# wearepal/qBOLD-VI

Measured on AMD Instinct MI355X. Metric: voxel-ELBO evals/sec, higher is better.
Workload: dtype f32; 1 GPU; 1048576 synthetic voxels/GPU x 11 tau, S=32 likelihood draws, K=70 KL draws, encoder U=60, L=2 (optimal.yaml), fused qbold_vi_fwd, tissue integral: table; encoder arithmetic: operands split in two f16 halves, three MFMA passes (hi.hi, hi.lo, lo.hi), f32 accumulate: float32-grade (~22 significant bits), |x| < 65504; sampling, forward model and ELBO sums: f32; global_voxels=1048576, parallelism=voxel-shard x1, collective=none

## Files before the change

### qbold_vi_amd/csrc/elbo_core.h

```cpp
#pragma once
#ifndef QB_PRIO_LIK
#define QB_PRIO_LIK 1
#endif
#ifndef QB_LIK_BARRIER
#define QB_LIK_BARRIER 2
#endif
#ifndef QB_GT_DEPTH
#define QB_GT_DEPTH 8
#endif
#ifndef QB_GT_DEPTH_LONG
#define QB_GT_DEPTH_LONG 2
#endif
#ifndef QB_X_DEPTH
#define QB_X_DEPTH 2
#endif
#ifndef QB_PRIO_KL
#define QB_PRIO_KL 2
#endif
#ifndef QB_PRIO_AFTER
#define QB_PRIO_AFTER 0
#endif

#include "qbold_dev.h"

// ... 76 lines not shown
    k.mask = mask;
}

template <int T, int SE, bool LITERAL>
__device__ __forceinline__ float sample_nll(const FwdLds* L, const QbDev& c, const VoxelLik<T>& k,
                                            float oef, float dbv) {
    const FwdVox fv = fwd_vox(c, oef, dbv);
    float s[T];
    if (SE >= 0) {
        constexpr int kSE = SE >= 0 ? SE : 0;
        float tis[T];
#pragma unroll
        for (int t = T - 1; t >= 0; --t) {
            const int m = (t < kSE && 2 * kSE - t < T) ? 2 * kSE - t : 0;
            const bool mirrored = t < kSE && 2 * kSE - t < T && c.full_model && c.taus[m] == -c.taus[t];
            if (mirrored) tis[t] = tis[m];
            else tis[t] = fwd_tissue<LITERAL>(L, c, fv, t);
            s[t] = fwd_mix(c, fv, tis[t], t);
        }
    } else {
#pragma unroll
        for (int t = 0; t < T; ++t) s[t] = fwd_signal<LITERAL>(L, c, fv, t);
    }
    const float inv_np = 1.0f / se_norm<T, SE>(c, s);
    float acc = 0.0f;
#pragma unroll
    for (int t = 0; t < T; ++t) {
        float yp = s[t] * inv_np;
        if (c.predict_log) yp = k.mask > 0.0f ? __logf(yp) : 0.0f;
        float r = (k.yt[t] - yp) * k.inv_s[t];
        if (c.use_student_t)
            acc += 0.5f * (c.st_df + 1.0f) * log1pf(r * r / c.st_df) - c.st_const;
        else
            acc = fmaf(0.5f * r, r, acc);
    }
    return acc + k.log_s_sum;
}

template <class LDS>
struct IsGtLds { static constexpr bool value = false; };
template <int T, int SE>
struct IsGtLds<GtLds<T, SE>> { static constexpr bool value = true; };

template <bool HELD>
struct GtStage {
    float4 kk;
    float bb;
};
template <>
struct GtStage<true> {
    float4 kk;
};

template <int T, int SE, class U = NoDrawRegs>
__device__ __forceinline__ float sample_sq_fast(const GtLds<T, SE>* L, const QbDev& c, const VoxelLik<T>& k,
                                                float sa, float sb, const U& u = U()) {
    static_assert(SE >= 0 && gtab_segs(T) > 0, "built for compile-time spin-echo protocols");
    static_assert(!U::kOn || !gtab_paired(T, SE), "held draw operands: built for the unpaired table");
    constexpr int NSEG = gtab_segs(T);
    FwdFast fv;
    float bb_se;
    if constexpr (U::kOn) {
        fv = fwd_fast_sig(u, sa, sb);
        bb_se = u.bb[SE];
    } else {
        fv = fwd_fast_sig(c, sa, sb);
        bb_se = L->blood_B[SE];
    }
    float acc = 0.0f;
    const float s_se = fmaf(fv.tissue_w, 1.0f, fv.blood_w * exp2f_(fv.ng * bb_se));
    const float inv_np = rcpf_(s_se + 1e-3f);
    const float lt = log2f_(fv.tissue_w * inv_np), lb = log2f_(fv.blood_w * inv_np);
    static_assert(QB_GT_OEF_MIN == QB_MIN_OEF && QB_GT_OEF_RANGE == QB_OEF_RANGE, "the table spans forward_transform's range");
    const float cg = fminf(sa * (float)NSEG, (float)NSEG - 0.0009765625f);
    const float f = __builtin_amdgcn_fractf(cg);
    const float4* row = L->gtab + (int)cg;
    {
        const float r = fmaf(-(s_se * inv_np), k.inv_s[SE], k.yt[SE]);
        acc = fmaf(r, r, acc);
    }
    constexpr int NA = T - 1 - SE, NB = (2 * SE - (T - 1)) > 0 ? 2 * SE - (T - 1) : 0, NE = NA + NB;
    auto score = [&](int t, float yh) {
        const float r = fmaf(-yh, k.inv_s[t], k.yt[t]);
        acc = fmaf(r, r, acc);
    };
    if constexpr (gtab_paired(T, SE)) {
        typedef float f32x2 __attribute__((ext_vector_type(2)));
        static_assert(NB == 0 && NA % 2 == 0, "paired table: every evaluated tau above the spin echo, in pairs");
        struct Stage {
            float4 A, B;
            f32x2 bb;
        };
        auto issue = [&](int p) -> Stage {
            Stage st;
            st.A = row[(2 * p) * NSEG];
            st.B = row[(2 * p + 1) * NSEG];
            st.bb = f32x2{L->blood_B[SE + 1 + 2 * p], L->blood_B[SE + 2 + 2 * p]};
            return st;
        };
        const f32x2 ff{f, f}, nd2{fv.nd, fv.nd}, ng2{fv.ng, fv.ng}, lt2{lt, lt}, lb2{lb, lb};
        auto finish = [&](int p, const Stage& st) {
            const f32x2 c0{st.A.x, st.A.y}, c1{st.A.z, st.A.w}, c2{st.B.x, st.B.y}, c3{st.B.z, st.B.w};
            const f32x2 F = __builtin_elementwise_fma(__builtin_elementwise_fma(__builtin_elementwise_fma(c3, ff, c2), ff, c1), ff, c0);
            const f32x2 e1 = __builtin_elementwise_fma(nd2, F, lt2), e2 = __builtin_elementwise_fma(ng2, st.bb, lb2);
            score(SE + 1 + 2 * p, exp2f_(e1.x) + exp2f_(e2.x));
            score(SE + 2 + 2 * p, exp2f_(e1.y) + exp2f_(e2.y));
        };
        constexpr int NP = NA / 2;
        constexpr int D = (QB_GT_DEPTH + 1) / 2 < NP ? (QB_GT_DEPTH + 1) / 2 : NP;
        Stage ring[D + 1];
#pragma unroll
        for (int e = 0; e < D; ++e) ring[e] = issue(e);
#pragma unroll
        for (int e = 0; e < NP; ++e) {
            if (e + D < NP) ring[(e + D) % (D + 1)] = issue(e + D);
            __builtin_amdgcn_sched_barrier(0);
            finish(e, ring[e % (D + 1)]);
            __builtin_amdgcn_sched_barrier(0);
        }
        return acc;
    } else {
        using Stage = GtStage<U::kOn>;
        auto issue = [&](int t) -> Stage {
            const int j = t > SE ? t - SE : SE - t;
            Stage st;
            st.kk = row[(j - 1) * NSEG];
            if constexpr (!U::kOn) st.bb = L->blood_B[t];
            return st;
        };
// ... 116 lines not shown
    bool whitened;
    if constexpr (LPV == 1) whitened = zk == nullptr && row_all(reach < QB_LOGIT_CLIP);
    else whitened = zk == nullptr && __all(reach < QB_LOGIT_CLIP);
    if (whitened) {
        const float dmu_o = q.mu_o - prior.mu_o, dmu_d = q.mu_d - prior.mu_d;
        const float d0 = dmu_o * prior.i_so, m00 = q.e_so * prior.i_so;
        const float d1 = fmaf(dmu_d, prior.i_sd, dmu_o * prior.i_bl);
        const float m10 = fmaf(q.c, prior.i_sd, q.e_so * prior.i_bl), m11 = q.e_sd * prior.i_sd;
        float s0 = 0.0f, s1 = 0.0f, s00 = 0.0f, s11 = 0.0f, s01 = 0.0f;
        for (int g = part; 4 * g < K; g += QB_LANES_PER_VOXEL) {
            float z[8];
            const int cnt = K - 4 * g < 4 ? K - 4 * g : 4;
            n_kl += cnt;
            normals8_unscaled(seed, vox, (uint32_t)g, STREAM_KL, cnt, z);
#pragma unroll
            for (int d = 0; d < 4; ++d) {
                s0 += z[2 * d];
                s1 += z[2 * d + 1];
                s00 = fmaf(z[2 * d], z[2 * d], s00);
                s11 = fmaf(z[2 * d + 1], z[2 * d + 1], s11);
                s01 = fmaf(z[2 * d], z[2 * d + 1], s01);
            }
        }
        s0 *= QB_BM_K;
        s1 *= QB_BM_K;
        s00 *= QB_BM_K * QB_BM_K;
        s11 *= QB_BM_K * QB_BM_K;
        s01 *= QB_BM_K * QB_BM_K;
        const float nk = (float)n_kl;
        const float quad = fmaf(fmaf(m00, m00, m10 * m10) - 1.0f, s00, fmaf(fmaf(m11, m11, -1.0f), s11, 2.0f * m10 * m11 * s01));
        const float lin = 2.0f * fmaf(fmaf(d0, m00, d1 * m10), s0, d1 * m11 * s1);
        return fmaf(nk, fmaf(d0, d0, d1 * d1), lin + quad);
    }
    for (int g = part; 4 * g < K; g += QB_LANES_PER_VOXEL) {
        const int cnt = K - 4 * g < 4 ? K - 4 * g : 4;
        n_kl += cnt;
        DrawQuad dq;
        if (!zk) dq.load(seed, vox, (uint32_t)g, STREAM_KL);
#pragma unroll 1
        for (int d = 0; d < cnt; ++d) {
            float z0, z1;
            if (zk) {
                z0 = zk[2 * (4 * g + d)];
                z1 = zk[2 * (4 * g + d) + 1];
            } else {
                dq.next(z0, z1);
            }
            kl_sum += kl_swr_diff(q, prior, z0, z1);
        }
    }
    return kl_sum;
}

template <int T, int SE, bool FAST, bool LITERAL, bool MIR, class LDS, class U = NoDrawRegs>
__device__ __forceinline__ float lik_draws(const LDS* L, const QbDev& c, const VoxelLik<T>& lik, const LogitMvn& q,
                                           int S, const float* __restrict__ zs, uint64_t seed, uint64_t vox, int part,
                                           int& n_lik, const U& u = U()) {
    static_assert(!U::kOn || (FAST && IsGtLds<LDS>::value), "held draw operands: the per-tau-table fast path");
    float nll_sum = 0.0f;
    const int calls = S > 4 * part ? (S - 4 * part + 15) / 16 : 0;
    const int last = calls > 0 ? S - 4 * (part + 4 * (calls - 1)) : 0;
    n_lik = calls > 0 ? 4 * (calls - 1) + (last < 4 ? last : 4) : 0;
    DrawQuad dq;
    uint32_t g = (uint32_t)part;
#pragma unroll 1
    for (int i = 0; i < n_lik; ++i) {
        float z0, z1;
        if (zs) {
            const int draw = 4 * (part + 4 * (i >> 2)) + (i & 3);
            z0 = zs[2 * draw];
            z1 = zs[2 * draw + 1];
        } else {
            if ((i & 3) == 0) {
                dq.load(seed, vox, g, STREAM_LIK);
                g += QB_LANES_PER_VOXEL;
            }
            dq.next(z0, z1);
        }
        float a, b, oef = 0.0f, dbv = 0.0f;
        reparam_logits(q, z0, z1, a, b);
        if constexpr (!(FAST && IsGtLds<LDS>::value)) forward_transform(a, b, oef, dbv);
        if constexpr (U::kOn) {
            nll_sum += sample_sq_fast<T, SE>(L, c, lik, sigmoidf_(a), sigmoidf_(b), u);
        } else if constexpr (FAST && IsGtLds<LDS>::value) {
            static_assert(!IsGtLds<LDS>::value || MIR, "the per-tau table scores merged mirror pairs");
            nll_sum += sample_sq_fast<T, SE>(L, c, lik, sigmoidf_(a), sigmoidf_(b));
        } else if constexpr (FAST) {
            nll_sum += sample_sq_fast<T, SE, MIR>(L, c, lik, oef, dbv);
        } else {
            nll_sum += sample_nll<T, SE, LITERAL>(L, c, lik, oef, dbv);
        }
    }
    return nll_sum;
}

__device__ __forceinline__ void share_sum(int p, float v, float& first, float& pair) {
    pair = (p & 1) ? pair + v : v;
    first = p == 1 ? pair : first;
}

template <int T, int SE, bool FAST, bool LITERAL, bool MIR = false, int LPV = QB_LANES_PER_VOXEL, bool DREGS = false,
          class LDS>
__device__ __forceinline__ void voxel_mc_sums(const LDS* L, const QbDev& c,
                                              const VoxelLik<T>& lik, const LogitMvn& q,
                                              const float* __restrict__ prior_row, int S, int K,
                                              const float* __restrict__ zs,
                                              const float* __restrict__ zk, uint64_t seed,
                                              uint64_t vox, int part, float& nll_sum,
                                              float& kl_sum) {
    static_assert(LPV == QB_LANES_PER_VOXEL || (LPV == 1 && FAST), "one lane per voxel: built for the fast path");
    static_assert(!DREGS || (LPV == 1 && IsGtLds<LDS>::value), "held draw operands: one lane per voxel on the per-tau table");
    nll_sum = 0.0f;
    kl_sum = 0.0f;
    int n_lik = 0, n_kl = 0;
    const float q_s_sum = q.s_o + q.s_d;
    __builtin_amdgcn_s_setprio(QB_PRIO_LIK);
    if constexpr (LPV == 1) {
        float first = 0.0f, pair = 0.0f;
        typename DrawRegsIf<DREGS, LikRegs<T, SE>>::type u;
        u.form(L, c);
#pragma unroll 1
        for (int p = 0; p < QB_LANES_PER_VOXEL; ++p) {
            const float sq = lik_draws<T, SE, FAST, LITERAL, MIR>(L, c, lik, q, S, zs, seed, vox, p, n_lik, u);
            share_sum(p, fmaf(0.5f, sq, (float)n_lik * lik.log_s_sum), first, pair);
        }
        nll_sum = first + pair;
    } else {
        const int calls = S > 4 * part ? (S - 4 * part + 15) / 16 : 0;
        const int last = calls > 0 ? S - 4 * (part + 4 * (calls - 1)) : 0;
        n_lik = calls > 0 ? 4 * (calls - 1) + (last < 4 ? last : 4) : 0;
        DrawQuad dq;
        uint32_t g = (uint32_t)part;
#pragma unroll 1
        for (int i = 0; i < n_lik; ++i) {
            float z0, z1;
            if (zs) {
                const int draw = 4 * (part + 4 * (i >> 2)) + (i & 3);
                z0 = zs[2 * draw];
                z1 = zs[2 * draw + 1];
            } else {
                if ((i & 3) == 0) {
                    dq.load(seed, vox, g, STREAM_LIK);
                    g += QB_LANES_PER_VOXEL;
                }
                dq.next(z0, z1);
            }
            float a, b, oef = 0.0f, dbv = 0.0f;
            reparam_logits(q, z0, z1, a, b);
            if constexpr (!(FAST && IsGtLds<LDS>::value)) forward_transform(a, b, oef, dbv);
            if constexpr (FAST && IsGtLds<LDS>::value) {
                static_assert(!IsGtLds<LDS>::value || MIR, "the per-tau table scores merged mirror pairs");
                nll_sum += sample_sq_fast<T, SE>(L, c, lik, sigmoidf_(a), sigmoidf_(b));
            } else if constexpr (FAST) {
                nll_sum += sample_sq_fast<T, SE, MIR>(L, c, lik, oef, dbv);
            } else {
                nll_sum += sample_nll<T, SE, LITERAL>(L, c, lik, oef, dbv);
            }
        }
        if (FAST) {
            nll_sum = fmaf(0.5f, nll_sum, (float)n_lik * lik.log_s_sum);
        }
    }
    float pv[5];
#pragma unroll
    for (int k = 0; k < 5; ++k) pv[k] = prior_row[k];
    const LogitMvn prior = make_mvn(pv);
    __builtin_amdgcn_s_setprio(QB_PRIO_KL);
    if constexpr (FAST) {
        LogitMvn qk;
        qk.mu_o = q.mu_o; qk.mu_d = q.mu_d; qk.c = q.c; qk.e_so = q.e_so; qk.e_sd = q.e_sd;
        qk.s_o = q_s_sum; qk.s_d = 0.0f;
        qk.i_so = rcpf_(q.e_so);
        qk.i_sd = rcpf_(q.e_sd);
        qk.i_bl = -(qk.i_so * qk.i_sd) * q.c;
        if constexpr (LPV == 1) {
            const float per_draw = (prior.s_o + prior.s_d) - q_s_sum;
            float first = 0.0f, pair = 0.0f;
// ... 79 lines not shown
```

### qbold_vi_amd/csrc/encoder_core.h

```cpp
#pragma once

#include "qbold_dev.h"

namespace qb {

typedef float f32x4 __attribute__((ext_vector_type(4)));

struct EncLayout {
    int T, U, L;
    int ksteps_first;
    int n_head;
    int head_tiles;
    int first_A, first_b;
    int blk0;
    int blk_stride;
    int head_A, head_b;
    int flag;
    int total;
};
enum { BLK_WC_A = 0, BLK_WC_B = 4096, BLK_R1_A = 4160, BLK_R1_B = 8256, BLK_R2_A = 8320,
       BLK_R2_B = 12416, BLK_G_A = 12480, BLK_G_B = 16576, BLK_FLOATS = 16640 };

__host__ __device__ constexpr inline EncLayout make_enc_layout(int T, int U, int L) {
    EncLayout e{};
// ... 119 lines not shown
            asm("v_fma_mixhi_f16 %0, %1, %2, %3 op_sel:[1,0,0] op_sel_hi:[1,0,0]" : "+v"(l) : "v"(h), "s"(nscale), "v"(sc[1]));
            hp[p] = h;
            lp[p] = l;
        }
        hi = __builtin_bit_cast(f16x8, hp);
        lo = __builtin_bit_cast(f16x8, lp);
#else
#pragma unroll
        for (int j = 0; j < 8; ++j) {
            const _Float16 h = (_Float16)v[j];
            hi[j] = h;
            lo[j] = (_Float16)((v[j] - (float)h) * QB_LO_SCALE);
        }
#endif
    }
}

struct ActFrag {
    f16x8 hi[2], lo[2];
};
#ifndef QB_AMAX_ASM
#define QB_AMAX_ASM 1
#endif
#define QB_SPLIT_MAX 65504.0f
__device__ __forceinline__ bool split_overflowed(float amax) { return !(amax <= QB_SPLIT_MAX); }

template <bool BF = false>
__device__ __forceinline__ ActFrag split_act(const f32x4 (&in)[4], float* amax = nullptr) {
    ActFrag f;
#pragma unroll
    for (int s = 0; s < 2; ++s) {
        const float v[8] = {in[2 * s][0], in[2 * s][1], in[2 * s][2], in[2 * s][3],
                            in[2 * s + 1][0], in[2 * s + 1][1], in[2 * s + 1][2], in[2 * s + 1][3]};
        if (!BF && amax) {
#pragma unroll
            for (int j = 0; j < 8; j += 2) {
#if QB_AMAX_ASM
                asm("v_max3_f32 %0, %0, |%1|, |%2|" : "+v"(*amax) : "v"(v[j]), "v"(v[j + 1]));
#else
                *amax = fmaxf(*amax, fmaxf(fabsf(v[j]), fabsf(v[j + 1])));
#endif
            }
        }
        split8<BF>(v, f.hi[s], f.lo[s]);
    }
    return f;
}

__device__ __forceinline__ f16x8 lds_frag(const float* __restrict__ A, int idx, int lane) {
    return *reinterpret_cast<const f16x8*>(reinterpret_cast<const unsigned char*>(A) + idx * 1024 +
                                           lane * 16);
}

template <int MT, int KS, bool BF = false>
__device__ __forceinline__ void dense_f16x3(const float* __restrict__ A,
                                            const float* __restrict__ bias, const f16x8 (&bhi)[KS],
                                            const f16x8 (&blo)[KS], f32x4 (&out)[MT], int lane) {
    const int g = lane >> 4;
    f32x4 cross[MT];
#pragma unroll
    for (int m = 0; m < MT; ++m) {
        out[m] = load4(bias + m * 16 + g * 4);
        cross[m] = f32x4{0.0f, 0.0f, 0.0f, 0.0f};
    }
    if constexpr (BF) {
        f16x8 whi = lds_frag(A, 0, lane);
#pragma unroll
        for (int s = 0; s < KS; ++s) {
#pragma unroll
            for (int m = 0; m < MT; ++m) {
                const int nxt = s * MT + m + 1;
                f16x8 nhi = whi;
                if (nxt < KS * MT) nhi = lds_frag(A, nxt * 2, lane);
                out[m] = QB_MFMA_BF16(as_bf16(whi), as_bf16(bhi[s]), out[m]);
                whi = nhi;
            }
        }
        return;
    }
    f16x8 whi = lds_frag(A, 0, lane), wlo = lds_frag(A, 1, lane);
    __builtin_amdgcn_s_setprio(3);
#pragma unroll
    for (int s = 0; s < KS; ++s) {
#pragma unroll
        for (int m = 0; m < MT; ++m) {
            const int nxt = s * MT + m + 1;
            f16x8 nhi = whi, nlo = wlo;
            if (nxt < KS * MT) {
                nhi = lds_frag(A, nxt * 2 + 0, lane);
                nlo = lds_frag(A, nxt * 2 + 1, lane);
            }
            out[m] = QB_MFMA_F16(whi, bhi[s], out[m]);
            cross[m] = QB_MFMA_F16(whi, blo[s], cross[m]);
            cross[m] = QB_MFMA_F16(wlo, bhi[s], cross[m]);
            whi = nhi;
            wlo = nlo;
            __builtin_amdgcn_sched_barrier(0);
        }
    }
    __builtin_amdgcn_s_setprio(QB_ENC_BASE_PRIO);
#pragma unroll
    for (int m = 0; m < MT; ++m) {
#pragma unroll
        for (int r = 0; r < 4; ++r) out[m][r] = fmaf(cross[m][r], QB_LO_UNSCALE, out[m][r]);
    }
}

template <bool BF = false>
__device__ __forceinline__ void dense64(const float* __restrict__ A, const float* __restrict__ bias,
                                        const f32x4 (&in)[4], f32x4 (&out)[4], int lane, float* amax = nullptr) {
    const ActFrag f = split_act<BF>(in, amax);
    dense_f16x3<4, 2, BF>(A, bias, f.hi, f.lo, out, lane);
}

template <int HT, bool BF = false>
__device__ __forceinline__ void dense_head(const float* __restrict__ A,
                                           const float* __restrict__ bias, const f32x4 (&in)[4],
                                           f32x4 (&out)[HT], int lane, float* amax = nullptr) {
    const ActFrag f = split_act<BF>(in, amax);
    dense_f16x3<HT, 2, BF>(A, bias, f.hi, f.lo, out, lane);
}

template <int T, int SE = -1>
__device__ __forceinline__ void normalise(const QbDev& c, const float (&x)[T], float (&n)[T]) {
    float cl[T];
#pragma unroll
    for (int t = 0; t < T; ++t) cl[t] = clampf_(x[t], 1e-2f, 1e8f);
    float den;
    if (SE >= 0) {
        den = cl[SE >= 0 ? SE : 0];
    } else {
        const int se = c.se_idx;
        float a = 0.0f, b = 0.0f, d = 0.0f;
#pragma unroll
        for (int t = 0; t < T; ++t) {
            a = (t == se - 1) ? cl[t] : a;
            b = (t == se) ? cl[t] : b;
            d = (t == se + 1) ? cl[t] : d;
        }
        den = c.multi_norm ? (a + b + d) / 3.0f : b;
    }
    const float inv_den = 1.0f / den;
#pragma unroll
    for (int t = 0; t < T; ++t) n[t] = QB_LN2 * log2f_(cl[t] * inv_den);
}

template <int T, bool BF = false>
__device__ __forceinline__ void dense_first(const float* __restrict__ A,
                                            const float* __restrict__ bias, const float (&n)[T],
                                            f32x4 (&out)[4], int lane) {
    static_assert(T <= 32, "first layer is a single K = 32 step");
    const int g = lane >> 4;
    float v[8];
#pragma unroll
    for (int j = 0; j < 8; ++j) {
        float x = 0.0f;
#pragma unroll
        for (int gg = 0; gg < 4; ++gg)
            if (8 * gg + j < T) x = (g == gg) ? n[(8 * gg + j < T) ? 8 * gg + j : 0] : x;
        v[j] = x;
    }
    f16x8 hi[1], lo[1];
    split8<BF>(v, hi[0], lo[0]);
    dense_f16x3<4, 1, BF>(A, bias, hi, lo, out, lane);
#pragma unroll
    for (int m = 0; m < 4; ++m) out[m] = relu4(out[m]);
}

__device__ __forceinline__ float med3f_(float v, float lo, float hi) { return __builtin_amdgcn_fmed3f(v, lo, hi); }

template <int T, int SE, bool BF = false>
__device__ __forceinline__ void first_operand(const float* __restrict__ xrow, int lane, f16x8& hi, f16x8& lo) {
    static_assert(T >= 8 && T <= 32 && SE >= 0 && SE < T, "one K = 32 step, windows of eight inside the row");
    constexpr int R = T % 8, GP = T / 8;
    const int g = lane >> 4;
    const float* w = xrow + (8 * g < T - 8 ? 8 * g : T - 8);
    float win[8];
#pragma unroll
    for (int j = 0; j < 8; ++j) win[j] = w[j];
    float se = xrow[SE];
    asm volatile("" : "+v"(se), "+v"(win[0]), "+v"(win[1]), "+v"(win[2]), "+v"(win[3]), "+v"(win[4]), "+v"(win[5]),
                      "+v"(win[6]), "+v"(win[7]));
    const float inv_den = 1.0f / med3f_(se, 1e-2f, 1e8f);
    float n[8], v[8];
#pragma unroll
    for (int j = 0; j < 8; ++j) n[j] = QB_LN2 * log2f_(med3f_(win[j], 1e-2f, 1e8f) * inv_den);
#pragma unroll
    for (int j = 0; j < 8; ++j) v[j] = (j < R && g == GP) ? n[j < R ? j + 8 - R : j] : n[j];
    split8<BF>(v, hi, lo);
}

template <bool BF = false>
__device__ __forceinline__ void dense_first_frag(const float* __restrict__ A, const float* __restrict__ bias,
                                                 const f16x8& hi, const f16x8& lo, f32x4 (&out)[4], int lane) {
    const f16x8 h[1] = {hi}, l[1] = {lo};
    dense_f16x3<4, 1, BF>(A, bias, h, l, out, lane);
#pragma unroll
    for (int m = 0; m < 4; ++m) out[m] = relu4(out[m]);
}

__device__ __forceinline__ ActFrag relu_frag(const ActFrag& f) {
    typedef uint32_t u32x4r __attribute__((ext_vector_type(4)));
    ActFrag o;
#pragma unroll
    for (int s = 0; s < 2; ++s) {
        const u32x4r h = __builtin_bit_cast(u32x4r, f.hi[s]), l = __builtin_bit_cast(u32x4r, f.lo[s]);
        u32x4r hp, lp;
#pragma unroll
        for (int p = 0; p < 4; ++p) {
            uint32_t neg;
            asm("v_pk_max_f16 %0, %1, 0" : "=v"(hp[p]) : "v"(h[p]));
            asm("v_pk_ashrrev_i16 %0, 15, %1 op_sel_hi:[0,1]" : "=v"(neg) : "v"(h[p]));
            lp[p] = l[p] & ~neg;
        }
        o.hi[s] = __builtin_bit_cast(f16x8, hp);
        o.lo[s] = __builtin_bit_cast(f16x8, lp);
    }
    return o;
}

__device__ __forceinline__ void gate_blend_f16x3(const float* __restrict__ W, const f16x8 (&bhi)[2],
                                                 const f16x8 (&blo)[2], const f32x4 (&skip)[4], f32x4 (&b)[4],
                                                 int lane) {
    const int g = lane >> 4;
    auto frag = [&](int n, int part) {
        const int m = n >> 2, s = (n >> 1) & 1, op = n & 1;
        return lds_frag(W + (op ? BLK_G_A : BLK_R2_A), (s * 4 + m) * 2 + part, lane);
    };
    f16x8 whi = frag(0, 0), wlo = frag(0, 1);
#pragma unroll
    for (int m = 0; m < 4; ++m) {
        f32x4 acc[2] = {load4(W + BLK_R2_B + m * 16 + g * 4), load4(W + BLK_G_B + m * 16 + g * 4)};
        f32x4 cross[2] = {f32x4{0.0f, 0.0f, 0.0f, 0.0f}, f32x4{0.0f, 0.0f, 0.0f, 0.0f}};
        __builtin_amdgcn_s_setprio(3);
#pragma unroll
        for (int n = 4 * m; n < 4 * m + 4; ++n) {
            const int s = (n >> 1) & 1, op = n & 1;
            f16x8 nhi = whi, nlo = wlo;
            if (n + 1 < 16) {
                nhi = frag(n + 1, 0);
                nlo = frag(n + 1, 1);
            }
            acc[op] = QB_MFMA_F16(whi, bhi[s], acc[op]);
            cross[op] = QB_MFMA_F16(whi, blo[s], cross[op]);
            cross[op] = QB_MFMA_F16(wlo, bhi[s], cross[op]);
            __builtin_amdgcn_sched_barrier(0);
            whi = nhi;
            wlo = nlo;
        }
        __builtin_amdgcn_s_setprio(QB_ENC_BASE_PRIO);
#pragma unroll
        for (int k = 0; k < 4; ++k) {
            const float r = fmaf(cross[0][k], QB_LO_UNSCALE, acc[0][k]);
            const float y = fmaf(cross[1][k], QB_LO_UNSCALE, acc[1][k]);
            const float gate = rcpf_(1.0f + exp2f_(y));
            b[m][k] = fmaf(gate, r - skip[m][k], skip[m][k]);
        }
    }
}

template <bool BF = false, bool NONNEG = false, bool FOLD = false>
__device__ __forceinline__ void block_stream2(const float* __restrict__ W, f32x4 (&b)[4],
                                              int lane, float* amax = nullptr) {
    f32x4 skip[4], t[4], r[4];
    const ActFrag fb = split_act<BF>(b, amax);
    dense_f16x3<4, 2, BF>(W + BLK_WC_A, W + BLK_WC_B, fb.hi, fb.lo, skip, lane);
#pragma unroll
    for (int m = 0; m < 4; ++m) skip[m] = relu4(skip[m]);
    if constexpr (NONNEG) {
        dense_f16x3<4, 2, BF>(W + BLK_R1_A, W + BLK_R1_B, fb.hi, fb.lo, t, lane);
    } else if constexpr (!BF) {
        const ActFrag fr = relu_frag(fb);
        dense_f16x3<4, 2, BF>(W + BLK_R1_A, W + BLK_R1_B, fr.hi, fr.lo, t, lane);
    } else {
#pragma unroll
        for (int m = 0; m < 4; ++m) b[m] = relu4(b[m]);
        dense64<BF>(W + BLK_R1_A, W + BLK_R1_B, b, t, lane);
    }
#pragma unroll
    for (int m = 0; m < 4; ++m) t[m] = relu4(t[m]);
    if constexpr (FOLD) {
        static_assert(!FOLD || !BF, "the folded gate ops: split-f16 encoder only");
        const ActFrag ft = split_act<false>(t, amax);
        gate_blend_f16x3(W, ft.hi, ft.lo, skip, b, lane);
        return;
    }
    dense64<BF>(W + BLK_R2_A, W + BLK_R2_B, t, r, lane, amax);
    dense64<BF>(W + BLK_G_A, W + BLK_G_B, r, t, lane, amax);
#pragma unroll
    for (int m = 0; m < 4; ++m) {
#pragma unroll
        for (int k = 0; k < 4; ++k) {
            const float gate = sigmoidf_(t[m][k]);
            b[m][k] = skip[m][k] * (1.0f - gate) + r[m][k] * gate;
        }
    }
}

template <bool BF = false>
__device__ __forceinline__ void block_stream1(const float* __restrict__ W, f32x4 (&a)[4],
                                              int lane, float* amax = nullptr) {
    f32x4 o[4];
    dense64<BF>(W + BLK_WC_A, W + BLK_WC_B, a, o, lane, amax);
#pragma unroll
    for (int m = 0; m < 4; ++m) a[m] = relu4(o[m]);
}

__device__ __forceinline__ void all_groups(float x, float (&v)[4]) {
    const unsigned u = __float_as_uint(x);
    const auto p = __builtin_amdgcn_permlane16_swap(u, u, false, false);
    const auto e = __builtin_amdgcn_permlane32_swap(p[0], p[0], false, false);
    const auto o = __builtin_amdgcn_permlane32_swap(p[1], p[1], false, false);
    v[0] = __uint_as_float(e[0]);
    v[1] = __uint_as_float(o[0]);
    v[2] = __uint_as_float(e[1]);
    v[3] = __uint_as_float(o[1]);
// ... 86 lines not shown
```

### qbold_vi_amd/csrc/qbold_dev.h

```cpp
#pragma once

#include <hip/hip_runtime.h>
#include <stdint.h>

#define QB_MAX_T 64
#define QB_TAB_SEG 256
#define QB_NNODE 129
#define QB_WAVE 64

struct QbDev {
    int T, se_idx, full_model, include_blood;
    int multi_norm, predict_log, use_student_t, tissue_mode;
#ifdef QBOLD_ABLATION
    int debug_skip;
#endif
    float dw_coef;
    float dw_coef_nohct;
    float e_te_r2t;
    float r2t_te;
    float m_bld_nb;
    float g0_c1;
    float g0_c2;
    float half_g2;
    float td2;
// ... 446 lines not shown
template <bool LITERAL>
__device__ __forceinline__ float fwd_signal(const FwdLds* L, const QbDev& c, const FwdVox& v,
                                            int t) {
    return fwd_mix(c, v, fwd_tissue<LITERAL>(L, c, v, t), t);
}

struct FwdFast {
    float ua, ub;
    float nd;
    float tissue_w;
    float blood_w;
    float ng;
};
__device__ __forceinline__ FwdFast fwd_fast(const QbDev& c, float oef, float dbv) {
    FwdFast v;
    const float dw = c.dw_coef * oef;
    v.ua = c.tauh0 * dw;
    v.ub = c.tauh_step * dw;
    v.nd = -QB_LOG2E * dbv;
    const float bw = c.bw_coef * dbv;
    v.tissue_w = (1.0f - bw) * c.e_te_r2t;
    v.blood_w = bw * c.bwe_coef;
    v.ng = c.ngk_l2e * (oef * oef);
    return v;
}
__device__ __forceinline__ FwdFast fwd_fast_sig(const QbDev& c, float sa, float sb) {
    FwdFast v;
    v.ua = v.ub = 0.0f;
    v.nd = fmaf(sb, c.nd_a, c.nd_b);
    v.tissue_w = fmaf(sb, c.tw_a, c.tw_b);
    v.blood_w = fmaf(sb, c.bv_a, c.bv_b);
    const float oef = fmaf(sa, QB_OEF_RANGE, QB_MIN_OEF);
    v.ng = c.ngk_l2e * (oef * oef);
    return v;
}
template <int T, int SE>
struct LikRegs {
    static constexpr bool kOn = true;
    float bb[T];
    float nd_a, nd_b, tw_a, tw_b, bv_a, bv_b, ngk_l2e, oef_range, oef_min;
    __device__ __forceinline__ void form(const GtLds<T, SE>* L, const QbDev& c) {
        constexpr int NB = (2 * SE - (T - 1)) > 0 ? 2 * SE - (T - 1) : 0;
#pragma unroll
        for (int t = 0; t < T; ++t)
            if (t >= SE || t < NB) bb[t] = vreg_(L->blood_B[t]);
        nd_a = vreg_(c.nd_a); nd_b = vreg_(c.nd_b);
        tw_a = vreg_(c.tw_a); tw_b = vreg_(c.tw_b);
        bv_a = vreg_(c.bv_a); bv_b = vreg_(c.bv_b);
        ngk_l2e = vreg_(c.ngk_l2e);
        oef_range = vreg_(QB_OEF_RANGE);
        oef_min = vreg_(QB_MIN_OEF);
    }
};
template <int T, int SE>
__device__ __forceinline__ FwdFast fwd_fast_sig(const LikRegs<T, SE>& u, float sa, float sb) {
    FwdFast v;
    v.ua = v.ub = 0.0f;
    v.nd = fmaf(sb, u.nd_a, u.nd_b);
    v.tissue_w = fmaf(sb, u.tw_a, u.tw_b);
    v.blood_w = fmaf(sb, u.bv_a, u.bv_b);
    const float oef = fmaf(sa, u.oef_range, u.oef_min);
    v.ng = u.ngk_l2e * (oef * oef);
    return v;
}
__device__ __forceinline__ float fwd_signal_fast(const FwdLds* L, const QbDev& c, const FwdFast& v,
                                                 int t) {
    const float u = fabsf(fmaf((float)t, v.ub, v.ua));
    const int i = (int)u;
    const float f = __builtin_amdgcn_fractf(u);
    const float4 k = L->tab[i];
    const float F = fmaf(fmaf(fmaf(k.w, f, k.z), f, k.y), f, k.x);
    const float e1 = exp2f_(v.nd * F);
    const float e2 = exp2f_(v.ng * c.blood_B[t]);
    return fmaf(v.tissue_w, e1, v.blood_w * e2);
}

__device__ __forceinline__ float wave_sum(float v) {
#pragma unroll
    for (int o = 32; o > 0; o >>= 1) v += __shfl_xor(v, o, 64);
    return v;
}

}
```

### qbold_vi_amd/csrc/vi_fwd_kernels.inc

```
#if QB_VI_FOLD
#define QB_VI_KERNEL(name) name##_fold
#define QB_VI_GATE_FOLD_ARG const float* __restrict__ gate_fold,
#define QB_VI_COPY_IMAGE(BLK) qb::copy_to_lds_fold<BLK, e.flag, e.blk0, NL>(lds_w, packed, gate_fold, e.total / 4)
#else
#define QB_VI_KERNEL(name) name
#define QB_VI_GATE_FOLD_ARG
#define QB_VI_COPY_IMAGE(BLK) qb::copy_to_lds<BLK>(lds_w, packed, e.total / 4)
#endif

template <int T, int NL, int SE, bool FAST, bool LITERAL, bool BF, bool GT = false, bool MIR = false, int BLK = kBlock>
__global__ __launch_bounds__(BLK) void QB_VI_KERNEL(vi_fwd_kernel)(
    QbDev c, const float4* __restrict__ g_tab, const float* __restrict__ packed, QB_VI_GATE_FOLD_ARG
    const float* __restrict__ x, const float* __restrict__ mask, const float* __restrict__ prior,
    int S, int K, uint64_t seed, int64_t voxel0, float* __restrict__ q_out,
    float2* __restrict__ nll_kl, double* __restrict__ partials, int64_t N) {
    constexpr EncLayout e = qb::make_enc_layout(T, 64, NL);
    static_assert(!GT || (FAST && SE >= 0 && qb::gtab_segs(T) > 0), "GT needs the fast path with a compile-time spin echo");
    static_assert(!MIR || (FAST && SE >= 0), "merged mirror pairs: fast path with a compile-time spin echo");
    static_assert(!QB_VI_FOLD || GT, "the folded gate ops: built for the per-tau-table fast path");
    constexpr bool kMir = GT || MIR;
    using Lds = typename ViLds<T, SE, GT>::type;
    extern __shared__ __align__(16) unsigned char smem[];
    float* lds_w = reinterpret_cast<float*>(smem);
    Lds* L = reinterpret_cast<Lds*>(smem + sizeof(float) * e.total);
    double* red = reinterpret_cast<double*>(smem + sizeof(float) * e.total + sizeof(Lds));
    constexpr int kWaves = BLK / 64;
    QB_VI_COPY_IMAGE(BLK);
    if constexpr (qb::IsGtLds<Lds>::value) {
        qb::gt_lds_fill(L, g_tab, c);
    } else {
        qb::fwd_lds_fill(L, g_tab, true);
        if (threadIdx.x < QB_MAX_T) L->blood_B[threadIdx.x] = c.blood_B[threadIdx.x];
    }
    __syncthreads();

    constexpr int HT = (5 + T + 15) / 16;
    const int lane0 = threadIdx.x & 63, wave = threadIdx.x >> 6;
    float s_nll = 0.0f, s_kl = 0.0f, s_m = 0.0f;
    const int64_t ntile = (N + 15) / 16;
    for (int64_t tile = (int64_t)blockIdx.x * kWaves + wave; tile < ntile;
         tile += (int64_t)gridDim.x * kWaves) {
        int lane = lane0;
        asm volatile("" : "+v"(lane));
        const int g = lane >> 4, i = lane & 15;
        const int64_t v = tile * 16 + i;
        const int64_t vc = v < N ? v : N - 1;
        float o[5 + T];
        float amax = lds_w[e.flag];
        {
            __builtin_amdgcn_s_setprio(QB_PRIO_TILE_START);
            float xv[T], nv[T];
#pragma unroll
            for (int t = 0; t < T; ++t) xv[t] = x[vc * T + t];
            qb::normalise<T, SE>(c, xv, nv);
            __builtin_amdgcn_s_setprio(2);
            f32x4 b[4];
            qb::dense_first<T, BF>(lds_w + e.first_A, lds_w + e.first_b, nv, b, lane);
            if (!QB_ABLATE(c, 1) && qb_phase_fence()) {
                qb::block_stream2<BF, true, QB_VI_FOLD>(lds_w + e.blk0, b, lane, &amax);
#pragma unroll
// ... 12 lines not shown
            for (int t = 0; t < T; ++t) xv[t] = xr[t];
#pragma unroll
            for (int k = 0; k < 5; ++k) qv[k] = o[k];
#pragma unroll
            for (int t = 0; t < T; ++t) sv[t] = o[5 + t];
            qb::VoxelLik<T> lik;
            qb::prepare_lik<T, SE, true, (FAST && SE >= 0), FAST, kMir>(c, xv, sv, FAST ? 1.0f : (mask ? mask[v] : 1.0f), lik);
            const qb::LogitMvn qm = qb::make_mvn(qv);
            if (g == 1 && q_out) {
#pragma unroll
                for (int k = 0; k < 5; ++k) q_out[v * 5 + k] = qv[k];
            }
            if (!BF && qb::split_overflowed(amax)) lik.log_s_sum = __builtin_nanf("");
            float nll_part, kl_part;
            qb::voxel_mc_sums<T, SE, FAST, LITERAL, kMir>(L, c, lik, qm, prior + v * 5, S, K, nullptr, nullptr, seed,
                                                    (uint64_t)(voxel0 + v), g, nll_part, kl_part);
            const float nll = qb::voxel_sum(nll_part) / (float)S;
            const float kl = K > 0 ? qb::voxel_sum(kl_part) / (float)K : 0.0f;
            if (g == 0) {
                const float* mp = mask;
                asm volatile("" : "+v"(mp));
                const float m = mp ? mp[v] : 1.0f;
                if (nll_kl) nll_kl[v] = make_float2(nll, kl);
                s_nll += nll * m;
                s_kl += m > 0.0f ? kl : 0.0f;
                s_m += m;
            }
        }
    }
    qb::block_partials(red, s_nll, s_kl, s_m, partials);
}

template <int T, int NL, int SE, bool BF, int BLK = kBlock>
__global__ __launch_bounds__(BLK) void QB_VI_KERNEL(vi_fwd_kernel_vox)(
    QbDev c, const float4* __restrict__ g_tab, const float* __restrict__ packed, QB_VI_GATE_FOLD_ARG
    const float* __restrict__ x, const float* __restrict__ mask, const float* __restrict__ prior,
    int S, int K, uint64_t seed, int64_t voxel0, float* __restrict__ q_out,
    float2* __restrict__ nll_kl, double* __restrict__ partials, int64_t N, int add_blocks) {
    constexpr EncLayout e = qb::make_enc_layout(T, 64, NL);
    static_assert(SE >= 0 && qb::gtab_segs(T) > 0, "built for the per-tau table with a compile-time spin echo");
    using Lds = qb::GtLds<T, SE>;
    extern __shared__ __align__(16) unsigned char smem[];
    float* lds_w = reinterpret_cast<float*>(smem);
    Lds* L = reinterpret_cast<Lds*>(smem + sizeof(float) * e.total);
    double* red = reinterpret_cast<double*>(smem + sizeof(float) * e.total + sizeof(Lds));
    constexpr int kWaves = BLK / 64;
    QB_VI_COPY_IMAGE(BLK);
    qb::gt_lds_fill(L, g_tab, c);
    __syncthreads();

    constexpr int HT = (5 + T + 15) / 16;
    constexpr bool kSlots = HT == 1 || BF || QB_VI_FOLD;
    constexpr bool kDrawRegs = BF || QB_VI_FOLD || !(T == 11 && NL == 2);
    const int lane0 = threadIdx.x & 63, wave = __builtin_amdgcn_readfirstlane(threadIdx.x >> 6);
    float s_nll = 0.0f, s_kl = 0.0f, s_m = 0.0f;
    auto uniform = [](float v) { return __uint_as_float(__builtin_amdgcn_readfirstlane(__float_as_uint(v))); };
    const int64_t ntile = (N + 63) / 64;
    for (int64_t tile = (int64_t)blockIdx.x * kWaves + wave; tile < ntile;
         tile += (int64_t)gridDim.x * kWaves) {
        float hs[4][HT][4], o[5 + T];
#pragma unroll
        for (int k = 0; k < 16 * HT; ++k) asm volatile("" : "=v"(hs[k / (4 * HT)][(k / 4) % HT][k % 4]));
        if constexpr (!kSlots) {
#pragma unroll
            for (int k = 0; k < 5 + T; ++k) o[k] = 0.0f;
        }
        unsigned long long hot = 0;
#pragma unroll 1
        for (int s = 0; s < 4; ++s) {
            int lane = lane0;
            asm volatile("" : "+v"(lane));
            const int i = lane & 15;
            const int64_t ve = tile * 64 + 16 * s + i;
            const int64_t vc = ve < N ? ve : N - 1;
            float amax = lds_w[e.flag];
            __builtin_amdgcn_s_setprio(QB_PRIO_TILE_START);
            qb::f16x8 fhi, flo;
            qb::first_operand<T, SE, BF>(x + vc * T, lane, fhi, flo);
            __builtin_amdgcn_s_setprio(2);
            f32x4 b[4];
            qb::dense_first_frag<BF>(lds_w + e.first_A, lds_w + e.first_b, fhi, flo, b, lane);
            if (!QB_ABLATE(c, 1) && qb_phase_fence()) {
                qb::block_stream2<BF, true, QB_VI_FOLD>(lds_w + e.blk0, b, lane, &amax);
#pragma unroll
                for (int l = 1; l < NL; ++l) qb::block_stream2<BF, false, QB_VI_FOLD>(lds_w + e.blk0 + l * e.blk_stride, b, lane, &amax);
            }
            f32x4 hd[HT];
            qb::dense_head<HT, BF>(lds_w + e.head_A, lds_w + e.head_b, b, hd, lane, &amax);
            if constexpr (kSlots) {
#pragma unroll
                for (int m = 0; m < HT; ++m) qb::keep_head_tile<BF>(s, hs[0][m], hs[1][m], hs[2][m], hs[3][m], hd[m]);
            } else {
                float os[5 + T];
                qb::gather_head<5 + T, HT>(hd, os);
#pragma unroll
                for (int k = 0; k < 5 + T; ++k) o[k] = (lane >> 4) == s ? os[k] : o[k];
            }
            if constexpr (!BF) {
                unsigned long long over = __ballot(qb::split_overflowed(amax));
                over |= over >> 32;
                over |= over >> 16;
                hot |= (over & 0xffffull) << (16 * s);
            }
        }
        __builtin_amdgcn_s_setprio(0);
        if constexpr (kSlots) {
            qb::transpose_heads<HT>(hs);
#pragma unroll
            for (int k = 0; k < 5 + T; ++k) o[k] = qb::head_row<HT>(hs, k);
        }
        int lane = lane0;
        asm volatile("" : "+v"(lane));
        const int64_t v = tile * 64 + lane;
        float t_nll = 0.0f, t_kl = 0.0f, t_m = 0.0f;
        if (v < N && !QB_ABLATE(c, 2) && qb_phase_fence()) {
            const float* xr = x + v * T;
            asm volatile("" : "+v"(xr));
            float xv[T], sv[T], qv[5];
#pragma unroll
            for (int t = 0; t < T; ++t) xv[t] = xr[t];
#pragma unroll
            for (int k = 0; k < 5; ++k) qv[k] = o[k];
#pragma unroll
            for (int t = 0; t < T; ++t) sv[t] = o[5 + t];
            qb::VoxelLik<T> lik;
            qb::prepare_lik<T, SE, true, true, true, true>(c, xv, sv, 1.0f, lik);
            const qb::LogitMvn qm = qb::make_mvn(qv);
            if (q_out) {
#pragma unroll
                for (int k = 0; k < 5; ++k) q_out[v * 5 + k] = qv[k];
            }
            if (!BF && ((hot >> lane) & 1)) lik.log_s_sum = __builtin_nanf("");
            float nll_sum, kl_sum;
            qb::voxel_mc_sums<T, SE, true, false, true, 1, kDrawRegs>(L, c, lik, qm, prior + v * 5, S, K, nullptr, nullptr,
                                                                      seed, (uint64_t)(voxel0 + v), 0, nll_sum, kl_sum);
            int Sd = S, Kd = K;
            asm volatile("" : "+s"(Sd), "+s"(Kd));
            const float nll = nll_sum / (float)Sd;
            const float kl = Kd > 0 ? kl_sum / (float)Kd : 0.0f;
            int lane_out = lane0;
            asm volatile("" : "+v"(lane_out));
            const int64_t vo = tile * 64 + lane_out;
            const float* mp = mask;
            asm volatile("" : "+v"(mp));
            const float m = mp ? mp[vo] : 1.0f;
            if (nll_kl) nll_kl[vo] = make_float2(nll, kl);
            t_nll = nll * m;
            t_kl = m > 0.0f ? kl : 0.0f;
            t_m = m;
        }
        s_nll = uniform(s_nll + qb::wave_sum(t_nll));
        s_kl = uniform(s_kl + qb::wave_sum(t_kl));
        s_m = uniform(s_m + qb::wave_sum(t_m));
    }
    const bool first = (threadIdx.x & 63) == 0;
    qb::block_partials(red, first ? s_nll : 0.0f, first ? s_kl : 0.0f, first ? s_m : 0.0f, partials,
                       (int)blockIdx.x < add_blocks);
}

#undef QB_VI_KERNEL
#undef QB_VI_GATE_FOLD_ARG
#undef QB_VI_COPY_IMAGE
```

Before: 2.828 billion voxel-ELBO evals/s.

## Address LDS tables via held 32-bit bases and unroll draws four per Philox call

Adds three default-on paths. The per-tau table is read through a 32-bit LDS base held in a scalar register, and encoder fragments are addressed from a per-lane base that advances by compile-time offsets. The likelihood loop now runs one Philox call per trip and consumes its four words in an unrolled inner loop, replacing the DrawQuad state machine. The aim is to cut 64-bit address arithmetic and loop overhead. In exchange it adds template plumbing and may raise register pressure.

```diff
diff --git a/qbold_vi_amd/csrc/elbo_core.h b/qbold_vi_amd/csrc/elbo_core.h
--- a/qbold_vi_amd/csrc/elbo_core.h
+++ b/qbold_vi_amd/csrc/elbo_core.h
@@ -152,9 +152,9 @@
     float4 kk;
 };
 
-template <int T, int SE, class U = NoDrawRegs>
+template <int T, int SE, class U = NoDrawRegs, class TB = NoDrawRegs>
 __device__ __forceinline__ float sample_sq_fast(const GtLds<T, SE>* L, const QbDev& c, const VoxelLik<T>& k,
-                                                float sa, float sb, const U& u = U()) {
+                                                float sa, float sb, const U& u = U(), const TB& tb = TB()) {
     static_assert(SE >= 0 && gtab_segs(T) > 0, "built for compile-time spin-echo protocols");
     static_assert(!U::kOn || !gtab_paired(T, SE), "held draw operands: built for the unpaired table");
     constexpr int NSEG = gtab_segs(T);
@@ -174,7 +174,7 @@
     static_assert(QB_GT_OEF_MIN == QB_MIN_OEF && QB_GT_OEF_RANGE == QB_OEF_RANGE, "the table spans forward_transform's range");
     const float cg = fminf(sa * (float)NSEG, (float)NSEG - 0.0009765625f);
     const float f = __builtin_amdgcn_fractf(cg);
-    const float4* row = L->gtab + (int)cg;
+    const auto row = gt_row(L, tb, (int)cg);
     {
         const float r = fmaf(-(s_se * inv_np), k.inv_s[SE], k.yt[SE]);
         acc = fmaf(r, r, acc);
@@ -397,17 +397,41 @@
     return kl_sum;
 }
 
-template <int T, int SE, bool FAST, bool LITERAL, bool MIR, class LDS, class U = NoDrawRegs>
+template <int T, int SE, bool FAST, bool LITERAL, bool MIR, bool QUAD = false, class LDS, class U = NoDrawRegs,
+          class TB = NoDrawRegs>
 __device__ __forceinline__ float lik_draws(const LDS* L, const QbDev& c, const VoxelLik<T>& lik, const LogitMvn& q,
                                            int S, const float* __restrict__ zs, uint64_t seed, uint64_t vox, int part,
-                                           int& n_lik, const U& u = U()) {
+                                           int& n_lik, const U& u = U(), const TB& tb = TB()) {
     static_assert(!U::kOn || (FAST && IsGtLds<LDS>::value), "held draw operands: the per-tau-table fast path");
+    static_assert(!TB::kOn || (FAST && IsGtLds<LDS>::value), "table base operand: the per-tau-table fast path");
     float nll_sum = 0.0f;
     const int calls = S > 4 * part ? (S - 4 * part + 15) / 16 : 0;
     const int last = calls > 0 ? S - 4 * (part + 4 * (calls - 1)) : 0;
     n_lik = calls > 0 ? 4 * (calls - 1) + (last < 4 ? last : 4) : 0;
+    uint32_t g = (uint32_t)part;
+    if constexpr (QUAD) {
+        static_assert(!QUAD || (FAST && IsGtLds<LDS>::value), "four draws per trip: the per-tau-table fast path");
+        if (!zs) {
+#pragma unroll 1
+            for (int k = 0; k < calls; ++k) {
+                const uint4 o = philox4x32_7(make_uint4((uint32_t)vox, (uint32_t)(vox >> 32), g, STREAM_LIK),
+                                             make_uint2((uint32_t)seed, (uint32_t)(seed >> 32)));
+                g += QB_LANES_PER_VOXEL;
+                const int cnt = k == calls - 1 ? (last < 4 ? last : 4) : 4;
+                const uint32_t w[4] = {o.x, o.y, o.z, o.w};
+#pragma unroll
+                for (int d = 0; d < 4; ++d) {
+                    if (d > 0 && d >= cnt) break;
+                    float z0, z1, a, b;
+                    box_muller16(w[d], z0, z1);
+                    reparam_logits(q, z0, z1, a, b);
+                    nll_sum += sample_sq_fast<T, SE>(L, c, lik, sigmoidf_(a), sigmoidf_(b), u, tb);
+                }
+            }
+            return nll_sum;
+        }
+    }
     DrawQuad dq;
-    uint32_t g = (uint32_t)part;
 #pragma unroll 1
     for (int i = 0; i < n_lik; ++i) {
         float z0, z1;
@@ -425,8 +449,8 @@
         float a, b, oef = 0.0f, dbv = 0.0f;
         reparam_logits(q, z0, z1, a, b);
         if constexpr (!(FAST && IsGtLds<LDS>::value)) forward_transform(a, b, oef, dbv);
-        if constexpr (U::kOn) {
-            nll_sum += sample_sq_fast<T, SE>(L, c, lik, sigmoidf_(a), sigmoidf_(b), u);
+        if constexpr (U::kOn || TB::kOn) {
+            nll_sum += sample_sq_fast<T, SE>(L, c, lik, sigmoidf_(a), sigmoidf_(b), u, tb);
         } else if constexpr (FAST && IsGtLds<LDS>::value) {
             static_assert(!IsGtLds<LDS>::value || MIR, "the per-tau table scores merged mirror pairs");
             nll_sum += sample_sq_fast<T, SE>(L, c, lik, sigmoidf_(a), sigmoidf_(b));
@@ -445,7 +469,7 @@
 }
 
 template <int T, int SE, bool FAST, bool LITERAL, bool MIR = false, int LPV = QB_LANES_PER_VOXEL, bool DREGS = false,
-          class LDS>
+          bool TBASE = false, bool QUAD = false, class LDS>
 __device__ __forceinline__ void voxel_mc_sums(const LDS* L, const QbDev& c,
                                               const VoxelLik<T>& lik, const LogitMvn& q,
                                               const float* __restrict__ prior_row, int S, int K,
@@ -455,6 +479,7 @@
                                               float& kl_sum) {
     static_assert(LPV == QB_LANES_PER_VOXEL || (LPV == 1 && FAST), "one lane per voxel: built for the fast path");
     static_assert(!DREGS || (LPV == 1 && IsGtLds<LDS>::value), "held draw operands: one lane per voxel on the per-tau table");
+    static_assert(!TBASE || (LPV == 1 && IsGtLds<LDS>::value), "table base operand: one lane per voxel on the per-tau table");
     nll_sum = 0.0f;
     kl_sum = 0.0f;
     int n_lik = 0, n_kl = 0;
@@ -464,10 +489,13 @@
         float first = 0.0f, pair = 0.0f;
         typename DrawRegsIf<DREGS, LikRegs<T, SE>>::type u;
         u.form(L, c);
+        typename DrawRegsIf<TBASE, GtTabBase<T, SE>>::type tb;
+        tb.form(L);
 #pragma unroll 1
         for (int p = 0; p < QB_LANES_PER_VOXEL; ++p) {
-            const float sq = lik_draws<T, SE, FAST, LITERAL, MIR>(L, c, lik, q, S, zs, seed, vox, p, n_lik, u);
+            const float sq = lik_draws<T, SE, FAST, LITERAL, MIR, QUAD>(L, c, lik, q, S, zs, seed, vox, p, n_lik, u, tb);
             share_sum(p, fmaf(0.5f, sq, (float)n_lik * lik.log_s_sum), first, pair);
+            if constexpr (QUAD) asm volatile("" : "+v"(first), "+v"(pair));
         }
         nll_sum = first + pair;
     } else {
diff --git a/qbold_vi_amd/csrc/encoder_core.h b/qbold_vi_amd/csrc/encoder_core.h
--- a/qbold_vi_amd/csrc/encoder_core.h
+++ b/qbold_vi_amd/csrc/encoder_core.h
@@ -195,11 +195,51 @@
                                            lane * 16);
 }
 
-template <int MT, int KS, bool BF = false>
+template <int ORIGIN>
+struct FragLane {
+    const float* img;
+    int lane;
+    uint32_t addr;
+    template <int NEW>
+    __device__ __forceinline__ FragLane<NEW> advance() const {
+        FragLane<NEW> n{img, lane, addr + (uint32_t)(NEW - ORIGIN)};
+        asm volatile("" : "+v"(n.addr));
+        return n;
+    }
+};
+__device__ __forceinline__ FragLane<0> frag_lane(const float* img, int lane) {
+    FragLane<0> f{img, lane, (uint32_t)(uintptr_t)img + (uint32_t)lane * 16u};
+    asm volatile("" : "+v"(f.addr));
+    return f;
+}
+template <bool ON>
+__device__ __forceinline__ auto lane_form(const float* img, int lane) {
+    if constexpr (ON) return frag_lane(img, lane);
+    else return lane;
+}
+template <int NEW>
+__device__ __forceinline__ int advance(int lane) { return lane; }
+template <int NEW, int ORIGIN>
+__device__ __forceinline__ FragLane<NEW> advance(const FragLane<ORIGIN>& f) { return f.template advance<NEW>(); }
+__device__ __forceinline__ int lane_of(int lane) { return lane; }
+template <int ORIGIN>
+__device__ __forceinline__ int lane_of(const FragLane<ORIGIN>& f) { return f.lane; }
+template <int ORIGIN>
+__device__ __forceinline__ f16x8 lds_frag(const float* __restrict__ A, int idx, const FragLane<ORIGIN>& f) {
+#if defined(__HIP_DEVICE_COMPILE__)
+    const uint32_t off = (uint32_t)(reinterpret_cast<const char*>(A) - reinterpret_cast<const char*>(f.img)) +
+                         (uint32_t)(idx * 1024 - ORIGIN);
+    return *reinterpret_cast<const __attribute__((address_space(3))) f16x8*>(f.addr + off);
+#else
+    return f16x8{};
+#endif
+}
+
+template <int MT, int KS, bool BF = false, class LN = int>
 __device__ __forceinline__ void dense_f16x3(const float* __restrict__ A,
                                             const float* __restrict__ bias, const f16x8 (&bhi)[KS],
-                                            const f16x8 (&blo)[KS], f32x4 (&out)[MT], int lane) {
-    const int g = lane >> 4;
+                                            const f16x8 (&blo)[KS], f32x4 (&out)[MT], LN lane) {
+    const int g = lane_of(lane) >> 4;
     f32x4 cross[MT];
 #pragma unroll
     for (int m = 0; m < MT; ++m) {
@@ -249,17 +289,17 @@
     }
 }
 
-template <bool BF = false>
+template <bool BF = false, class LN = int>
 __device__ __forceinline__ void dense64(const float* __restrict__ A, const float* __restrict__ bias,
-                                        const f32x4 (&in)[4], f32x4 (&out)[4], int lane, float* amax = nullptr) {
+                                        const f32x4 (&in)[4], f32x4 (&out)[4], LN lane, float* amax = nullptr) {
     const ActFrag f = split_act<BF>(in, amax);
     dense_f16x3<4, 2, BF>(A, bias, f.hi, f.lo, out, lane);
 }
 
-template <int HT, bool BF = false>
+template <int HT, bool BF = false, class LN = int>
 __device__ __forceinline__ void dense_head(const float* __restrict__ A,
                                            const float* __restrict__ bias, const f32x4 (&in)[4],
-                                           f32x4 (&out)[HT], int lane, float* amax = nullptr) {
+                                           f32x4 (&out)[HT], LN lane, float* amax = nullptr) {
     const ActFrag f = split_act<BF>(in, amax);
     dense_f16x3<HT, 2, BF>(A, bias, f.hi, f.lo, out, lane);
 }
@@ -333,9 +373,9 @@
     split8<BF>(v, hi, lo);
 }
 
-template <bool BF = false>
+template <bool BF = false, class LN = int>
 __device__ __forceinline__ void dense_first_frag(const float* __restrict__ A, const float* __restrict__ bias,
-                                                 const f16x8& hi, const f16x8& lo, f32x4 (&out)[4], int lane) {
+                                                 const f16x8& hi, const f16x8& lo, f32x4 (&out)[4], LN lane) {
     const f16x8 h[1] = {hi}, l[1] = {lo};
     dense_f16x3<4, 1, BF>(A, bias, h, l, out, lane);
 #pragma unroll
@@ -362,10 +402,11 @@
     return o;
 }
 
+template <class LN = int>
 __device__ __forceinline__ void gate_blend_f16x3(const float* __restrict__ W, const f16x8 (&bhi)[2],
                                                  const f16x8 (&blo)[2], const f32x4 (&skip)[4], f32x4 (&b)[4],
-                                                 int lane) {
-    const int g = lane >> 4;
+                                                 LN lane) {
+    const int g = lane_of(lane) >> 4;
     auto frag = [&](int n, int part) {
         const int m = n >> 2, s = (n >> 1) & 1, op = n & 1;
         return lds_frag(W + (op ? BLK_G_A : BLK_R2_A), (s * 4 + m) * 2 + part, lane);
@@ -402,9 +443,9 @@
     }
 }
 
-template <bool BF = false, bool NONNEG = false, bool FOLD = false>
+template <bool BF = false, bool NONNEG = false, bool FOLD = false, class LN = int>
 __device__ __forceinline__ void block_stream2(const float* __restrict__ W, f32x4 (&b)[4],
-                                              int lane, float* amax = nullptr) {
+                                              LN lane, float* amax = nullptr) {
     f32x4 skip[4], t[4], r[4];
     const ActFrag fb = split_act<BF>(b, amax);
     dense_f16x3<4, 2, BF>(W + BLK_WC_A, W + BLK_WC_B, fb.hi, fb.lo, skip, lane);
diff --git a/qbold_vi_amd/csrc/qbold_dev.h b/qbold_vi_amd/csrc/qbold_dev.h
--- a/qbold_vi_amd/csrc/qbold_dev.h
+++ b/qbold_vi_amd/csrc/qbold_dev.h
@@ -522,6 +522,33 @@
         oef_min = vreg_(QB_MIN_OEF);
     }
 };
+struct LdsRows {
+    uint32_t addr;
+    __device__ __forceinline__ float4 operator[](int k) const {
+#if defined(__HIP_DEVICE_COMPILE__)
+        typedef float f32x4r __attribute__((ext_vector_type(4)));
+        const f32x4r r = reinterpret_cast<const __attribute__((address_space(3))) f32x4r*>(addr)[k];
+        return make_float4(r.x, r.y, r.z, r.w);
+#else
+        return make_float4(0.0f, 0.0f, 0.0f, 0.0f);
+#endif
+    }
+};
+template <int T, int SE>
+struct GtTabBase {
+    static constexpr bool kOn = true;
+    uint32_t base;
+    __device__ __forceinline__ void form(const GtLds<T, SE>* L) {
+        base = (uint32_t)(uintptr_t)L->gtab;
+        asm volatile("" : "+s"(base));
+    }
+};
+template <int T, int SE>
+__device__ __forceinline__ const float4* gt_row(const GtLds<T, SE>* L, const NoDrawRegs&, int i) { return L->gtab + i; }
+template <int T, int SE>
+__device__ __forceinline__ LdsRows gt_row(const GtLds<T, SE>*, const GtTabBase<T, SE>& tb, int i) {
+    return LdsRows{tb.base + ((uint32_t)i << 4)};
+}
 template <int T, int SE>
 __device__ __forceinline__ FwdFast fwd_fast_sig(const LikRegs<T, SE>& u, float sa, float sb) {
     FwdFast v;
diff --git a/qbold_vi_amd/csrc/vi_fwd_kernels.inc b/qbold_vi_amd/csrc/vi_fwd_kernels.inc
--- a/qbold_vi_amd/csrc/vi_fwd_kernels.inc
+++ b/qbold_vi_amd/csrc/vi_fwd_kernels.inc
@@ -6,6 +6,16 @@
 #define QB_VI_KERNEL(name) name
 #define QB_VI_GATE_FOLD_ARG
 #define QB_VI_COPY_IMAGE(BLK) qb::copy_to_lds<BLK>(lds_w, packed, e.total / 4)
+#endif
+
+#ifndef QB_VI_TAB_BASE
+#define QB_VI_TAB_BASE 1
+#endif
+#ifndef QB_VI_FRAG_BASE
+#define QB_VI_FRAG_BASE 1
+#endif
+#ifndef QB_VI_QUAD_DRAWS
+#define QB_VI_QUAD_DRAWS 1
 #endif
 
 template <int T, int NL, int SE, bool FAST, bool LITERAL, bool BF, bool GT = false, bool MIR = false, int BLK = kBlock>
@@ -124,6 +134,12 @@
     constexpr int HT = (5 + T + 15) / 16;
     constexpr bool kSlots = HT == 1 || BF || QB_VI_FOLD;
     constexpr bool kDrawRegs = BF || QB_VI_FOLD || !(T == 11 && NL == 2);
+    constexpr bool kQuadDraws = QB_VI_QUAD_DRAWS && (BF || NL == 1 || (!QB_VI_FOLD && T == 11));
+    constexpr bool kTabBase = QB_VI_TAB_BASE;
+    constexpr bool kFragBase = QB_VI_FRAG_BASE && (BF ? (T == 24 && NL == 2) : QB_VI_FOLD != 0);
+    static_assert(NL <= 2, "the blocks are written out: at most two");
+    static_assert(!kFragBase || (4 * qb::BLK_G_A + 15 * 1024 < 65536 && 4 * e.blk0 <= 65536),
+                  "FragLane windows: the first layer, a block, the heads");
     const int lane0 = threadIdx.x & 63, wave = __builtin_amdgcn_readfirstlane(threadIdx.x >> 6);
     float s_nll = 0.0f, s_kl = 0.0f, s_m = 0.0f;
     auto uniform = [](float v) { return __uint_as_float(__builtin_amdgcn_readfirstlane(__float_as_uint(v))); };
@@ -150,15 +166,16 @@
             qb::f16x8 fhi, flo;
             qb::first_operand<T, SE, BF>(x + vc * T, lane, fhi, flo);
             __builtin_amdgcn_s_setprio(2);
-            f32x4 b[4];
-            qb::dense_first_frag<BF>(lds_w + e.first_A, lds_w + e.first_b, fhi, flo, b, lane);
+            f32x4 b[4], hd[HT];
+            const auto f0 = qb::lane_form<kFragBase>(lds_w, lane);
+            qb::dense_first_frag<BF>(lds_w + e.first_A, lds_w + e.first_b, fhi, flo, b, f0);
+            const auto f1 = qb::advance<4 * e.blk0>(f0);
             if (!QB_ABLATE(c, 1) && qb_phase_fence()) {
-                qb::block_stream2<BF, true, QB_VI_FOLD>(lds_w + e.blk0, b, lane, &amax);
-#pragma unroll
-                for (int l = 1; l < NL; ++l) qb::block_stream2<BF, false, QB_VI_FOLD>(lds_w + e.blk0 + l * e.blk_stride, b, lane, &amax);
-            }
-            f32x4 hd[HT];
-            qb::dense_head<HT, BF>(lds_w + e.head_A, lds_w + e.head_b, b, hd, lane, &amax);
+                qb::block_stream2<BF, true, QB_VI_FOLD>(lds_w + e.blk0, b, f1, &amax);
+                if constexpr (NL == 2)
+                    qb::block_stream2<BF, false, QB_VI_FOLD>(lds_w + e.blk0 + e.blk_stride, b, qb::advance<4 * (e.blk0 + e.blk_stride)>(f1), &amax);
+            }
+            qb::dense_head<HT, BF>(lds_w + e.head_A, lds_w + e.head_b, b, hd, qb::advance<4 * e.head_A>(f1), &amax);
             if constexpr (kSlots) {
 #pragma unroll
                 for (int m = 0; m < HT; ++m) qb::keep_head_tile<BF>(s, hs[0][m], hs[1][m], hs[2][m], hs[3][m], hd[m]);
@@ -204,8 +221,8 @@
             }
             if (!BF && ((hot >> lane) & 1)) lik.log_s_sum = __builtin_nanf("");
             float nll_sum, kl_sum;
-            qb::voxel_mc_sums<T, SE, true, false, true, 1, kDrawRegs>(L, c, lik, qm, prior + v * 5, S, K, nullptr, nullptr,
-                                                                      seed, (uint64_t)(voxel0 + v), 0, nll_sum, kl_sum);
+            qb::voxel_mc_sums<T, SE, true, false, true, 1, kDrawRegs, kTabBase, kQuadDraws>(L, c, lik, qm, prior + v * 5, S, K, nullptr,
+                                                                            nullptr, seed, (uint64_t)(voxel0 + v), 0, nll_sum, kl_sum);
             int Sd = S, Kd = K;
             asm volatile("" : "+s"(Sd), "+s"(Kd));
             const float nll = nll_sum / (float)Sd;
```

Result: no change. 2.852 billion voxel-ELBO evals/s, median of 6 (+0.9%).
